# foundation-model-stack/fms-fsdp

Measured on AMD Instinct MI355X. Metric: tokens/sec (aggregate), higher is better.
Workload: dtype bf16; 1 GPU; model=llama2_7b, global_batch=2, seq_len=4096, parallelism=hsdp1

## Files before the change

fms_fsdp_amd/models/llama.py:

```python

import math
import os
from dataclasses import dataclass


import torch
import torch.nn as nn

from fms_fsdp_amd import ops


@dataclass
class LlamaConfig:
    src_vocab_size: int = 32000
    emb_dim: int = 4096
    nheads: int = 32
    kvheads: int = 0
    nlayers: int = 32
    hidden_grow_factor: float = 8 / 3
    multiple_of: int = 256
    max_expected_seq_len: int = 4096
    rope_theta: float = 10000.0
    norm_eps: float = 1e-6

# ... 101 lines not shown
        v = v.view(b, s, self.kvheads, self.head_dim)
        q, k = ops.rope_apply(q, k, cos, sin)
        if cache is not None:
            import torch.nn.functional as F
            if cache.get("k") is not None:
                k = torch.cat([cache["k"], k], dim=1)
                v = torch.cat([cache["v"], v], dim=1)
            cache["k"], cache["v"] = k, v
            o = F.scaled_dot_product_attention(
                q.transpose(1, 2), k.transpose(1, 2), v.transpose(1, 2),
                is_causal=(s == k.shape[1]),
                enable_gqa=(self.kvheads != self.nheads)).transpose(1, 2)
        else:
            o = ops.attention_causal(q, k, v, doc_mask=doc_mask)
        return self._project_out(o.reshape(b, s, -1), residual, b, s)

    def reset_parameters(self):
        for lin in (self.qkv, self.proj):
            nn.init.trunc_normal_(lin.weight, mean=0.0, std=0.02)


class SwiGLU(nn.Module):
    def __init__(self, cfg: LlamaConfig):
        super().__init__()
        self.hidden_dim = cfg.hidden_dim
        self.wg1 = nn.Linear(cfg.emb_dim, 2 * cfg.hidden_dim, bias=False)
        self.w2 = nn.Linear(cfg.hidden_dim, cfg.emb_dim, bias=False)
        self.wg1.weight._direct_wgrad = True
        self.w2.weight._direct_wgrad = True

    def forward(self, x, residual=None):
        if getattr(self, "_disable_fused_residual", False):
            gu = self.wg1(x)
            h = ops.swiglu(gu)
            out = self.w2(h)
            return out if residual is None else out + residual.view_as(out)
        gu = ops.linear_flat(x, self.wg1.weight)
        h = ops.swiglu(gu)
        return ops.linear_flat(h, self.w2.weight, residual)

    def reset_parameters(self):
        for lin in (self.wg1, self.w2):
            nn.init.trunc_normal_(lin.weight, mean=0.0, std=0.02)


class LlamaBlock(nn.Module):

    def __init__(self, cfg: LlamaConfig):
        super().__init__()
        self.attn_norm = RMSNorm(cfg.emb_dim, cfg.norm_eps)
        self.attn = Attention(cfg)
        self.mlp_norm = RMSNorm(cfg.emb_dim, cfg.norm_eps)
        self.mlp = SwiGLU(cfg)

    def forward(self, x, cos, sin, cache=None, doc_mask=None):
        if cache is None and getattr(self, "_ac_enabled", False) \
                and torch.is_grad_enabled():
            return torch.utils.checkpoint.checkpoint(
                self._forward_impl, x, cos, sin, None, doc_mask,
                use_reentrant=False)
        return self._forward_impl(x, cos, sin, cache, doc_mask)

    def _forward_impl(self, x, cos, sin, cache=None, doc_mask=None):
        h = self.attn(self.attn_norm(x), cos, sin, cache, residual=x,
                      doc_mask=doc_mask)
        return self.mlp(self.mlp_norm(h), residual=h)

    def reset_parameters(self):
        for m in (self.attn_norm, self.attn, self.mlp_norm, self.mlp):
            m.reset_parameters()


class Llama(nn.Module):
    def __init__(self, cfg: LlamaConfig):
        super().__init__()
        self.config = cfg
        self.embedding = nn.Embedding(cfg.src_vocab_size, cfg.emb_dim)
        self.rot_emb = RotaryEmbedding(cfg.head_dim, cfg.max_expected_seq_len, cfg.rope_theta)
        self.layers = nn.ModuleList([LlamaBlock(cfg) for _ in range(cfg.nlayers)])
        self.norm = RMSNorm(cfg.emb_dim, cfg.norm_eps)
        self.lm_head = nn.Linear(cfg.emb_dim, cfg.src_vocab_size, bias=False)
        self.doc_mask_token = None

    def forward(self, tokens, labels=None, include_embeds=False,
                doc_mask=None):
        b, s = tokens.shape
        if doc_mask is None and self.doc_mask_token is not None:
            doc_mask = ops.doc_mask_from_tokens(tokens, self.doc_mask_token)
        x = self.embedding(tokens)
        cos, sin = self.rot_emb.get(s, x.device)
        for layer in self.layers:
            x = layer(x, cos, sin, doc_mask=doc_mask)
        x = self.norm(x)
        if labels is not None:
            loss = ops.linear_cross_entropy(x, self.lm_head.weight, labels)
            return (loss, x) if include_embeds else loss
        logits = self.lm_head(x)
        return (logits, x) if include_embeds else logits

    @torch.no_grad()
    def generate(self, input_ids, max_new_tokens, temperature=1.0,
                 do_sample=True, include_embeds=False):
        b, s0 = input_ids.shape
        caches = [{} for _ in self.layers]
        tokens = input_ids
        embeds = []
        cur = input_ids
        pos = 0
        for step in range(max_new_tokens):
            x = self.embedding(cur)
            total = pos + cur.shape[1]
            cos, sin = self.rot_emb.get(total, x.device)
            cos_c, sin_c = cos[pos:total], sin[pos:total]
            for layer, cache in zip(self.layers, caches):
                x = layer(x, cos_c, sin_c, cache)
            x = self.norm(x)
            h_last = x[:, -1:]
            logits = self.lm_head(h_last)[:, -1]
            if do_sample:
                probs = torch.softmax(logits.float() / temperature, dim=-1)
                nxt = torch.multinomial(probs, 1)
            else:
                nxt = logits.argmax(-1, keepdim=True)
            embeds.append(h_last)
            tokens = torch.cat([tokens, nxt], dim=1)
            pos = total
            cur = nxt
        if include_embeds:
            return tokens, torch.cat(embeds, dim=1)
        return tokens

    def reset_root_parameters(self):
        nn.init.trunc_normal_(self.embedding.weight, mean=0.0, std=0.02)
# ... 11 lines not shown
```

fms_fsdp_amd/ops/__init__.py:

```python

import os
from typing import NamedTuple

import torch

from . import reference


_C = None
_C_err = None
try:
    from fms_fsdp_amd import _C
except ImportError as e:
    _C_err = e


def _require_ext(op):
    if _C is None:
        raise RuntimeError(
            f"fms_fsdp_amd._C HIP extension is required for {op} on GPU but "
            f"could not be imported ({_C_err}). Build it with "
            f"`python setup.py build_ext --inplace` (PYTORCH_ROCM_ARCH=gfx950)."
        )
    return _C


class _RMSNormFn(torch.autograd.Function):
    @staticmethod
    def forward(ctx, x, weight, eps):
        ext = _require_ext("rmsnorm")
        x2d = x.contiguous().view(-1, x.shape[-1])
        y, rinv = ext.rmsnorm_fwd(x2d, weight, eps)
        ctx.save_for_backward(x2d, weight, rinv)
        ctx.shape = x.shape
        return y.view(x.shape)

    @staticmethod
    def backward(ctx, dy):
        x2d, weight, rinv = ctx.saved_tensors
        dx, dw = _C.rmsnorm_bwd(dy.contiguous().view_as(x2d), x2d, weight,
                                rinv, None)
        return dx.view(ctx.shape), dw.to(weight.dtype), None


def rmsnorm(x, weight, eps=1e-6):
    if x.is_cuda and x.dtype != torch.float32:
        if x.dtype == torch.float16:
            return _RMSNormFn.apply(x.bfloat16(), weight.bfloat16(),
                                    eps).half()
        return _RMSNormFn.apply(x, weight, eps)
    return reference.rmsnorm(x, weight, eps)


class _AddRMSNormFn(torch.autograd.Function):

    @staticmethod
    def forward(ctx, x, res, weight, eps):
        ext = _require_ext("add_rmsnorm")
        x2d = x.contiguous().view(-1, x.shape[-1])
        r2d = res.contiguous().view_as(x2d)
        y, s, rinv = ext.add_rmsnorm_fwd(x2d, r2d, weight, eps)
        ctx.save_for_backward(s, weight, rinv)
        ctx.shape = x.shape
        return y.view(x.shape), s.view(x.shape)

    @staticmethod
    def backward(ctx, dy, ds):
        s, weight, rinv = ctx.saved_tensors
        dx, dw = _C.rmsnorm_bwd(dy.contiguous().view_as(s), s, weight, rinv,
                                ds.contiguous().view_as(s))
        dx = dx.view(ctx.shape)
        return dx, dx, dw.to(weight.dtype), None


def add_rmsnorm(x, res, weight, eps=1e-6):
    if x.is_cuda and x.dtype != torch.float32:
        if x.dtype == torch.float16:
            y, s = _AddRMSNormFn.apply(x.bfloat16(), res.bfloat16(),
                                       weight.bfloat16(), eps)
            return y.half(), s.half()
        return _AddRMSNormFn.apply(x, res, weight, eps)
    s = (x.float() + res.float()).to(x.dtype)
    return reference.rmsnorm(s, weight, eps), s


def _row_view_ok(t):
    return (t.dim() == 4 and t.stride(3) == 1 and t.stride(2) == t.shape[3]
            and t.stride(1) >= t.shape[2] * t.shape[3]
            and t.stride(0) == t.shape[1] * t.stride(1))


def _as_row_view(t):
    return t if _row_view_ok(t) else t.contiguous()


class _RoPEFn(torch.autograd.Function):
    @staticmethod
    def forward(ctx, q, k, cos, sin):
        ext = _require_ext("rope")
        cos = cos.float().contiguous()
        sin = sin.float().contiguous()
        qo, ko = ext.rope_fwd(_as_row_view(q), _as_row_view(k), cos, sin,
                              False)
        ctx.save_for_backward(cos, sin)
# ... 477 lines not shown
```

fms_fsdp_amd/ops/hip/attention.hip:

```cpp
#include <cstdlib>
#include <cstring>

#include "common.h"
#include "attn_sched.h"
#include "attn_ws.h"

typedef __attribute__((ext_vector_type(8))) __bf16 bf16x8v;
typedef __attribute__((ext_vector_type(16))) float f32x16;
typedef __attribute__((ext_vector_type(4))) float f32x4v;

union U8 {
  bf16x8v v;
  unsigned u[4];
  bf16x8 s;
};

__device__ __forceinline__ unsigned pack2(float lo, float hi) {
  return ((unsigned)(unsigned short)f2bf(hi) << 16) |
         (unsigned short)f2bf(lo);
}

__device__ __forceinline__ bf16x8v pack_pT_chunk(const float* p) {
  unsigned w01 = pack2(p[0], p[1]);
  unsigned w23 = pack2(p[2], p[3]);
// ... 288 lines not shown
    if (act1) {
      const unsigned pvbase = pvb[cur] + 1024;
      U2x64 fr[2][2];
      tr_issue4<0, 128, 512, 640>(pvbase, fr[0][0], fr[0][1]);
#pragma unroll
      for (int t = 0; t < NT; ++t) {
        const int pp = t & 1;
        if (t + 1 < NT) {
          if (t + 1 == 1)
            tr_issue4<4096, 4096 + 128, 4096 + 512, 4096 + 640>(
                pvbase, fr[1][0], fr[1][1]);
          else if (t + 1 == 2)
            tr_issue4<8192, 8192 + 128, 8192 + 512, 8192 + 640>(
                pvbase, fr[0][0], fr[0][1]);
          else
            tr_issue4<12288, 12288 + 128, 12288 + 512, 12288 + 640>(
                pvbase, fr[1][0], fr[1][1]);
          tr_wait<4>(fr[pp][0], fr[pp][1]);
        } else {
          tr_wait<0>(fr[pp][0], fr[pp][1]);
        }
        accO[t] = __builtin_amdgcn_mfma_f32_32x32x16_bf16(fr[pp][0].v, pb1_0,
                                                          accO[t], 0, 0, 0);
        accO[t] = __builtin_amdgcn_mfma_f32_32x32x16_bf16(fr[pp][1].v, pb1_1,
                                                          accO[t], 0, 0, 0);
      }
    }
    __syncthreads();
    cur ^= 1;
  }

  const float inv_l = 1.f / l_run;
  short* op = og + ((long long)b * S * H + (long long)h) * D +
              (long long)my_q * qrow_stride;
#pragma unroll
  for (int t = 0; t < NT; ++t) {
#pragma unroll
    for (int g = 0; g < 4; ++g) {
      const int dv0 = t * 32 + 8 * g + 4 * hb;
      bf16x4 w;
#pragma unroll
      for (int j = 0; j < 4; ++j)
        w.v[j] = f2bf(accO[t][g * 4 + j] * inv_l);
      *(bf16x4*)(op + dv0) = w;
    }
  }
  if (hb == 0)
    lseg[((long long)bh) * S + my_q] =
        (m_run + __log2f(l_run)) * 0.6931471805599453f;
}
#undef KLDS
#undef VLDS

__global__ void attn_bwd_delta_kernel(const short* __restrict__ dog,
                                      const short* __restrict__ og,
                                      float* __restrict__ delta,
                                      int D, int S, int H, long long rows) {
  const long long row = ((long long)blockIdx.x * blockDim.x + threadIdx.x) / 64;
  if (row >= rows) return;
  const int lane = threadIdx.x & 63;
  const short* dop = dog + row * D;
  const short* op = og + row * D;
  float acc = 0.f;
  for (int i = lane * 2; i < D; i += 128) {
    acc += bf2f(dop[i]) * bf2f(op[i]) + bf2f(dop[i + 1]) * bf2f(op[i + 1]);
  }
  acc = wave_reduce_sum(acc);
  if (lane == 0) {
    const long long b = row / ((long long)S * H);
    const int si = (int)((row / H) % S);
    const int hi = (int)(row % H);
    delta[(b * H + hi) * (long long)S + si] = acc;
  }
}

template <int D>
__global__ __launch_bounds__(256, 2) void attn_bwd_dq_kernel(
    const short* __restrict__ kg, const short* __restrict__ dsw,
    short* __restrict__ dqg, int B, int S, int H, int KVH, int sched,
    int ws_tiled) {
  constexpr int KVB = 32;
  constexpr int NT = D / 32;
  extern __shared__ __attribute__((aligned(16))) char smem[];
  constexpr int KIMGB = KVB * D * 2;
  constexpr int SIMGB = KVB * 128 * 2;
#define KIMG(buf) (smem + ((buf) ? KIMGB + SIMGB : 0))
#define SIMG(buf) (smem + KIMGB + ((buf) ? KIMGB + SIMGB : 0))

  const int lane = threadIdx.x & 63;
  const int wid = threadIdx.x >> 6;
  const int col = lane & 31;
  const int hb = lane >> 5;

  const AttnWork wk = attn_sched_map(blockIdx.x, S / 128, B * H, sched, false);
  const int bh = __builtin_amdgcn_readfirstlane(wk.bh);
  const int b = bh / H;
  const int h = bh % H;
  const int kvh = h / (H / KVH);
  const int q0 = __builtin_amdgcn_readfirstlane(wk.tile) * 128;
  const int qw = q0 + wid * 32;
  const int my_q = qw + col;

  const long long qrow_stride = (long long)H * D;
  const long long krow_stride = (long long)KVH * D;
  const short* kbase = kg + ((long long)b * S * KVH + (long long)kvh) * D;
  const short* dsbase = dsw + (long long)bh * S * S + q0;

  f32x16 accDQ[NT];
#pragma unroll
  for (int t = 0; t < NT; ++t) accDQ[t] = (f32x16)(0.f);

  const int ntiles = (q0 + 128 + KVB - 1) / KVB;
  const int t256 = threadIdx.x;
  const int skey = t256 & 31;
  const int sgrp = t256 >> 5;
  const int skd0 = sgrp * (D / 8);
  const short* kp_s = kbase + (long long)skey * krow_stride + skd0;
  const long long kstep = (long long)KVB * krow_stride;
  const short* sp_s =
      ws_tiled ? dsw + (long long)bh * S * S +
                     (long long)(q0 / 32 + (sgrp >> 1)) * 1024 +
// ... 855 lines not shown
  attn_bwd_dkv_keylane_kernel<D, OUT, false, true>                            \
      <<<grid, 256, lds_dkv, stream>>>(                                       \
          (const short*)do_, (const short*)q, (const short*)k,                \
          (const short*)v, lse, delta_ws, dk, dv, (short*)nullptr, B, S, H,   \
          KVH, scale, vstride, dvstride, sched, 0, doc_end)
  if (out_bf16)
    DKV_DOC_LAUNCH(true);
  else
    DKV_DOC_LAUNCH(false);
#undef DKV_DOC_LAUNCH
  const int lds_dq = 2 * (32 * D * 2 + 32 * D * 2);
  attn_bwd_dq_recompute_kernel<D, true><<<grid, 256, lds_dq, stream>>>(
      (const short*)do_, (const short*)q, (const short*)k, (const short*)v,
      lse, delta_ws, (short*)dq, B, S, H, KVH, scale, vstride, sched,
      doc_start);
}

extern "C" {

long long attn_bwd_ws_limit(long long bytes) {
  const long long prev = attn_ws_limit_get();
  if (bytes >= 0) g_attn_ws_limit = bytes;
  return prev;
}

int attn_sched_mode(int mode) {
  const int prev = attn_sched_get();
  if (mode >= 0) g_attn_sched = mode;
  return prev;
}

int attn_dkv_mode(int mode) {
  const int prev = attn_dkv_get();
  if (mode >= 0) g_attn_dkv = mode;
  return prev;
}

void launch_attn_fwd(const void* q, const void* k, const void* v, void* o,
                     float* lse, int B, int S, int H, int KVH, int D,
                     float scale, long long vstride, hipStream_t stream) {
  const unsigned grid = (unsigned)(S / 128) * (unsigned)(B * H);
  const int sched = attn_sched_get();
  const int lds = 3 * 64 * D * 2;
  if (D == 128)
    attn_fwd_kernel<128><<<grid, 256, lds, stream>>>(
        (const short*)q, (const short*)k, (const short*)v, (short*)o, lse, B,
        S, H, KVH, scale, vstride, sched);
  else
    attn_fwd_kernel<64><<<grid, 256, lds, stream>>>(
        (const short*)q, (const short*)k, (const short*)v, (short*)o, lse, B,
        S, H, KVH, scale, vstride, sched);
}

void launch_attn_bwd(const void* do_, const void* q, const void* k,
                     const void* v, const void* o, const float* lse, void* dq,
                     void* dk, void* dv, float* delta_ws, void* ds_ws,
                     int B, int S, int H,
                     int KVH, int D, float scale, int out_bf16,
                     long long vstride, long long dvstride,
                     hipStream_t stream) {
  const long long rows = (long long)B * S * H;
  attn_bwd_delta_kernel<<<(int)((rows * 64 + 255) / 256), 256, 0, stream>>>(
      (const short*)do_, (const short*)o, delta_ws, D, S, H, rows);
  if (D == 128)
    attn_bwd_launch<128>(do_, q, k, v, lse, dq, dk, dv, delta_ws, ds_ws, B, S,
                         H, KVH, scale, out_bf16, vstride, dvstride, stream);
  else
    attn_bwd_launch<64>(do_, q, k, v, lse, dq, dk, dv, delta_ws, ds_ws, B, S,
                        H, KVH, scale, out_bf16, vstride, dvstride, stream);
}

void launch_attn_fwd_doc(const void* q, const void* k, const void* v, void* o,
                         float* lse, const int* doc_start, int B, int S,
                         int H, int KVH, int D, float scale,
                         long long vstride, hipStream_t stream) {
  const unsigned grid = (unsigned)(S / 128) * (unsigned)(B * H);
  const int sched = attn_sched_get();
  const int lds = 3 * 64 * D * 2;
  if (D == 128)
    attn_fwd_kernel<128, true><<<grid, 256, lds, stream>>>(
        (const short*)q, (const short*)k, (const short*)v, (short*)o, lse, B,
        S, H, KVH, scale, vstride, sched, doc_start);
  else
    attn_fwd_kernel<64, true><<<grid, 256, lds, stream>>>(
        (const short*)q, (const short*)k, (const short*)v, (short*)o, lse, B,
        S, H, KVH, scale, vstride, sched, doc_start);
}

void launch_attn_bwd_doc(const void* do_, const void* q, const void* k,
                         const void* v, const void* o, const float* lse,
                         void* dq, void* dk, void* dv, float* delta_ws,
                         const int* doc_start, const int* doc_end, int B,
                         int S, int H, int KVH, int D, float scale,
                         int out_bf16, long long vstride, long long dvstride,
                         hipStream_t stream) {
  const long long rows = (long long)B * S * H;
  attn_bwd_delta_kernel<<<(int)((rows * 64 + 255) / 256), 256, 0, stream>>>(
      (const short*)do_, (const short*)o, delta_ws, D, S, H, rows);
  if (D == 128)
    attn_bwd_doc_launch<128>(do_, q, k, v, lse, dq, dk, dv, delta_ws,
                             doc_start, doc_end, B, S, H, KVH, scale,
                             out_bf16, vstride, dvstride, stream);
  else
    attn_bwd_doc_launch<64>(do_, q, k, v, lse, dq, dk, dv, delta_ws,
                            doc_start, doc_end, B, S, H, KVH, scale,
                            out_bf16, vstride, dvstride, stream);
}

}
```

fms_fsdp_amd/ops/hip/bindings.cpp:

```cpp
#include <torch/extension.h>
#include <c10/hip/HIPStream.h>
#include <hip/hip_runtime_api.h>

#include <string>
#include <tuple>
#include <vector>

#include "attn_ws.h"

using torch::Tensor;

extern "C" {
void launch_rmsnorm_fwd(const void*, const void*, void*, float*, int, int,
                        float, hipStream_t);
void launch_rmsnorm_bwd(const void*, const void*, const void*, const float*,
                        const void*, void*, float*, int, int, hipStream_t);
void launch_add_rmsnorm_fwd(const void*, const void*, const void*, void*,
                            void*, float*, int, int, float, hipStream_t);
void launch_rope(const void*, void*, const float*, const float*, int, int,
                 int, int, int, long long, long long, hipStream_t);
void launch_swiglu_fwd(const void*, void*, long long, int, hipStream_t);
void launch_swiglu_bwd(const void*, const void*, void*, long long, int,
                       hipStream_t);
void launch_ce_fwd_bwd(void*, const long long*, float*, const float*,
                       long long, int, int, hipStream_t);
void launch_adamw(float*, const void*, int, float*, float*, void*, int,
                  long long, float, float, float, float, float, float, float,
                  const float*, hipStream_t);
void launch_sqnorm(const void*, int, float*, long long, hipStream_t);
void launch_attn_fwd(const void*, const void*, const void*, void*, float*,
                     int, int, int, int, int, float, long long, hipStream_t);
void launch_attn_bwd(const void*, const void*, const void*, const void*,
                     const void*, const float*, void*, void*, void*, float*,
                     void*, int, int, int, int, int, float, int,
                     long long, long long, hipStream_t);
void launch_attn_fwd_doc(const void*, const void*, const void*, void*, float*,
                         const int*, int, int, int, int, int, float,
                         long long, hipStream_t);
void launch_attn_bwd_doc(const void*, const void*, const void*, const void*,
                         const void*, const float*, void*, void*, void*,
                         float*, const int*, const int*, int, int, int, int,
                         int, float, int, long long, long long, hipStream_t);
int attn_sched_mode(int);
int attn_dkv_mode(int);
long long attn_bwd_ws_limit(long long);
void launch_cconv_fwd(const void*, const void*, const float*, void*, int,
                      int, int, int, hipStream_t);
void launch_cconv_bwd(const void*, const void*, const void*, const float*,
                      void*, void*, float*, float*, int, int, int, int,
                      hipStream_t);
int launch_gemm_nt(const void*, const void*, void*, int, int, int,
                   hipStream_t);
void launch_segsum_exp_fwd(const float*, void*, long long, int, hipStream_t);
void launch_segsum_exp_bwd(const void*, const float*, float*, long long, int,
                           hipStream_t);
void launch_ssd_prep_fwd(const void*, const float*, const float*, float*,
                         float*, long long, int, int, long long, hipStream_t);
void launch_ssd_prep_bwd(const float*, const float*, const void*,
                         const float*, const float*, void*, float*, float*,
                         long long, int, int, long long, long long,
                         hipStream_t);
void launch_ssd_xdt_fwd(const void*, const float*, const float*, void*, void*,
                        long long, int, int, int, long long, hipStream_t);
void launch_ssd_xdt_bwd(const void*, const void*, const void*, const float*,
                        const float*, void*, float*, float*, long long, int,
                        int, int, long long, long long, hipStream_t);
void launch_ssd_sl_fwd(const float*, const void*, void*, long long, int, int,
                       int, hipStream_t);
void launch_ssd_sl_bwd(const void*, const void*, const float*, void*, float*,
                       long long, int, int, int, hipStream_t);
void launch_ssd_ygate_fwd(const void*, const void*, const float*, const void*,
                          const float*, const void*, void*, long long, int,
                          int, int, int, long long, long long, hipStream_t);
void launch_ssd_ygate_bwd(const void*, const void*, const void*, const float*,
                          const void*, const float*, const void*, void*,
                          void*, float*, void*, float*, void*, long long, int,
                          int, int, int, long long, long long, long long,
                          long long, hipStream_t);
}

static hipStream_t cur_stream() {
  return c10::hip::getCurrentHIPStream().stream();
}

#define CHECK_BF16_CONTIG(t)                                        \
  TORCH_CHECK(t.scalar_type() == torch::kBFloat16, #t " must be bf16"); \
  TORCH_CHECK(t.is_contiguous(), #t " must be contiguous");

std::tuple<Tensor, Tensor> rmsnorm_fwd(Tensor x, Tensor w, double eps) {
  CHECK_BF16_CONTIG(x);
  CHECK_BF16_CONTIG(w);
  const int rows = x.size(0), H = x.size(1);
  TORCH_CHECK(H % 8 == 0, "H must be divisible by 8");
  auto y = torch::empty_like(x);
  auto rinv = torch::empty({rows}, x.options().dtype(torch::kFloat32));
  launch_rmsnorm_fwd(x.data_ptr(), w.data_ptr(), y.data_ptr(),
                     rinv.data_ptr<float>(), rows, H, (float)eps,
                     cur_stream());
  return {y, rinv};
}

std::tuple<Tensor, Tensor> rmsnorm_bwd(Tensor dy, Tensor x, Tensor w,
                                       Tensor rinv,
                                       c10::optional<Tensor> dextra) {
  CHECK_BF16_CONTIG(dy);
  CHECK_BF16_CONTIG(x);
  CHECK_BF16_CONTIG(w);
  TORCH_CHECK(x.dim() == 2 && dy.sizes() == x.sizes(),
              "dy and x must be (rows, H)");
  const int rows = x.size(0), H = x.size(1);
  TORCH_CHECK(H % 8 == 0, "H must be divisible by 8");
  TORCH_CHECK(w.numel() == H, "w must have H elements");
  TORCH_CHECK(rinv.scalar_type() == torch::kFloat32 && rinv.is_contiguous() &&
                  rinv.numel() == rows,
              "rinv must be fp32 with one element per row");
  if (dextra.has_value()) {
    TORCH_CHECK(dextra->scalar_type() == torch::kBFloat16 &&
                    dextra->is_contiguous() && dextra->sizes() == x.sizes(),
                "dextra must have x's shape and dtype");
  }
  auto dx = torch::empty_like(x);
  auto dw = torch::zeros({H}, x.options().dtype(torch::kFloat32));
  launch_rmsnorm_bwd(dy.data_ptr(), x.data_ptr(), w.data_ptr(),
                     rinv.data_ptr<float>(),
                     dextra.has_value() ? dextra->data_ptr() : nullptr,
                     dx.data_ptr(), dw.data_ptr<float>(), rows, H,
                     cur_stream());
  return {dx, dw};
}

std::tuple<Tensor, Tensor, Tensor> add_rmsnorm_fwd(Tensor x, Tensor res,
                                                   Tensor w, double eps) {
  CHECK_BF16_CONTIG(x);
  CHECK_BF16_CONTIG(res);
  const int rows = x.size(0), H = x.size(1);
  auto y = torch::empty_like(x);
  auto s_out = torch::empty_like(x);
  auto rinv = torch::empty({rows}, x.options().dtype(torch::kFloat32));
  launch_add_rmsnorm_fwd(x.data_ptr(), res.data_ptr(), w.data_ptr(),
                         y.data_ptr(), s_out.data_ptr(),
                         rinv.data_ptr<float>(), rows, H, (float)eps,
                         cur_stream());
  return {y, s_out, rinv};
}

static long long row_stride4(const Tensor& t) {
  TORCH_CHECK(t.scalar_type() == torch::kBFloat16, "expected bf16");
  TORCH_CHECK(t.dim() == 4 && t.stride(3) == 1 &&
                  t.stride(2) == t.size(3) &&
                  t.stride(1) >= t.size(2) * t.size(3) &&
                  t.stride(0) == t.size(1) * t.stride(1),
              "expected row-contiguous (b,s,h,d) view");
  return (long long)t.stride(1);
}

std::tuple<Tensor, Tensor> rope_fwd(Tensor q, Tensor k, Tensor cos,
                                    Tensor sin, bool conj) {
  TORCH_CHECK(cos.scalar_type() == torch::kFloat32 && cos.is_contiguous());
  const int b = q.size(0), s = q.size(1), h = q.size(2), d = q.size(3);
  const int kvh = k.size(2);
  const long long qs = row_stride4(q), ks = row_stride4(k);
  TORCH_CHECK((d / 2) % 4 == 0, "head_dim/2 must be divisible by 4");
  auto qo = torch::empty({b, s, h, d}, q.options());
  auto ko = torch::empty({b, s, kvh, d}, k.options());
  launch_rope(q.data_ptr(), qo.data_ptr(), cos.data_ptr<float>(),
              sin.data_ptr<float>(), b, s, h, d, conj, qs,
              (long long)h * d, cur_stream());
  launch_rope(k.data_ptr(), ko.data_ptr(), cos.data_ptr<float>(),
              sin.data_ptr<float>(), b, s, kvh, d, conj, ks,
              (long long)kvh * d, cur_stream());
  return {qo, ko};
}

void rope_into(Tensor src, Tensor dst, Tensor cos, Tensor sin, bool conj) {
  const int b = src.size(0), s = src.size(1), h = src.size(2),
            d = src.size(3);
  const long long is = row_stride4(src), os = row_stride4(dst);
  TORCH_CHECK(dst.size(2) == h && dst.size(3) == d);
  launch_rope(src.data_ptr(), dst.data_ptr(), cos.data_ptr<float>(),
              sin.data_ptr<float>(), b, s, h, d, conj, is, os,
              cur_stream());
// ... 126 lines not shown
std::tuple<Tensor, Tensor> attn_fwd(Tensor q, Tensor k, Tensor v) {
  CHECK_BF16_CONTIG(q);
  CHECK_BF16_CONTIG(k);
  const long long vs = row_stride4(v);
  const int b = q.size(0), s = q.size(1), h = q.size(2), d = q.size(3);
  const int kvh = k.size(2);
  TORCH_CHECK(d == 64 || d == 128, "head_dim must be 64 or 128");
  TORCH_CHECK(s % 128 == 0, "seq len must be a multiple of 128");
  auto o = torch::empty_like(q);
  auto lse = torch::empty({b, h, s}, q.options().dtype(torch::kFloat32));
  const float scale = 1.f / sqrtf((float)d);
  launch_attn_fwd(q.data_ptr(), k.data_ptr(), v.data_ptr(), o.data_ptr(),
                  lse.data_ptr<float>(), b, s, h, kvh, d, scale, vs,
                  cur_stream());
  return {o, lse};
}

std::tuple<Tensor, Tensor, Tensor> attn_bwd(Tensor do_, Tensor q, Tensor k,
                                            Tensor v, Tensor o, Tensor lse,
                                            c10::optional<Tensor> dv_out) {
  CHECK_BF16_CONTIG(do_);
  const long long vs = row_stride4(v);
  const int b = q.size(0), s = q.size(1), h = q.size(2), d = q.size(3);
  const int kvh = k.size(2);
  auto dq = torch::empty_like(q);
  const bool out_bf16 = (kvh == h);
  auto opts = q.options().dtype(out_bf16 ? torch::kBFloat16 : torch::kFloat32);
  auto dk = out_bf16 ? torch::empty({b, s, kvh, d}, opts)
                     : torch::zeros({b, s, kvh, d}, opts);
  Tensor dv;
  long long dvs = (long long)kvh * d;
  if (dv_out.has_value() && out_bf16) {
    dv = *dv_out;
    dvs = row_stride4(dv);
  } else {
    dv = out_bf16 ? torch::empty({b, s, kvh, d}, opts)
                  : torch::zeros({b, s, kvh, d}, opts);
  }
  auto delta = torch::empty({b, h, s}, q.options().dtype(torch::kFloat32));
  Tensor ds_ws;
  if (attn_bwd_use_workspace(b, h, s, attn_bwd_ws_limit(-1)))
    ds_ws = torch::empty({(long long)b * h, (long long)s, (long long)s},
                         q.options());
  const float scale = 1.f / sqrtf((float)d);
  launch_attn_bwd(do_.data_ptr(), q.data_ptr(), k.data_ptr(), v.data_ptr(),
                  o.data_ptr(), lse.data_ptr<float>(), dq.data_ptr(),
                  dk.data_ptr(), dv.data_ptr(), delta.data_ptr<float>(),
                  ds_ws.defined() ? ds_ws.data_ptr() : nullptr, b, s,
                  h, kvh, d, scale, out_bf16 ? 1 : 0, vs, dvs, cur_stream());
  if (out_bf16) return {dq, dk, dv};
  return {dq, dk.to(torch::kBFloat16), dv.to(torch::kBFloat16)};
}

static void check_doc_array(const Tensor& t, const Tensor& q,
                            const char* name) {
  TORCH_CHECK(t.scalar_type() == torch::kInt32, name, " must be int32");
  TORCH_CHECK(t.is_contiguous(), name, " must be contiguous");
  TORCH_CHECK(t.dim() == 2 && t.size(0) == q.size(0) && t.size(1) == q.size(1),
              name, " must have shape (b, s)");
  TORCH_CHECK(t.device() == q.device(), name, " must be on q's device");
}

std::tuple<Tensor, Tensor> attn_fwd_doc(Tensor q, Tensor k, Tensor v,
                                        Tensor doc_start) {
  CHECK_BF16_CONTIG(q);
  CHECK_BF16_CONTIG(k);
  const long long vs = row_stride4(v);
  const int b = q.size(0), s = q.size(1), h = q.size(2), d = q.size(3);
  const int kvh = k.size(2);
  TORCH_CHECK(d == 64 || d == 128, "head_dim must be 64 or 128");
  TORCH_CHECK(s % 128 == 0, "seq len must be a multiple of 128");
  check_doc_array(doc_start, q, "doc_start");
  auto o = torch::empty_like(q);
  auto lse = torch::empty({b, h, s}, q.options().dtype(torch::kFloat32));
  const float scale = 1.f / sqrtf((float)d);
  launch_attn_fwd_doc(q.data_ptr(), k.data_ptr(), v.data_ptr(), o.data_ptr(),
                      lse.data_ptr<float>(), doc_start.data_ptr<int>(), b, s,
                      h, kvh, d, scale, vs, cur_stream());
  return {o, lse};
}

std::tuple<Tensor, Tensor, Tensor> attn_bwd_doc(
    Tensor do_, Tensor q, Tensor k, Tensor v, Tensor o, Tensor lse,
    c10::optional<Tensor> dv_out, Tensor doc_start, Tensor doc_end) {
  CHECK_BF16_CONTIG(do_);
  const long long vs = row_stride4(v);
  const int b = q.size(0), s = q.size(1), h = q.size(2), d = q.size(3);
  const int kvh = k.size(2);
  check_doc_array(doc_start, q, "doc_start");
  check_doc_array(doc_end, q, "doc_end");
  auto dq = torch::empty_like(q);
  const bool out_bf16 = (kvh == h);
  auto opts = q.options().dtype(out_bf16 ? torch::kBFloat16 : torch::kFloat32);
  auto dk = out_bf16 ? torch::empty({b, s, kvh, d}, opts)
                     : torch::zeros({b, s, kvh, d}, opts);
  Tensor dv;
  long long dvs = (long long)kvh * d;
  if (dv_out.has_value() && out_bf16) {
    dv = *dv_out;
    dvs = row_stride4(dv);
  } else {
    dv = out_bf16 ? torch::empty({b, s, kvh, d}, opts)
                  : torch::zeros({b, s, kvh, d}, opts);
  }
  auto delta = torch::empty({b, h, s}, q.options().dtype(torch::kFloat32));
  const float scale = 1.f / sqrtf((float)d);
// ... 247 lines not shown
  check_nq(dacs, x.size(0) / Q * H, Q, "dacs");
  check_head_vec(Dp, H, "D");
}

Tensor ssd_ygate_fwd(Tensor ydiag, Tensor yoff, Tensor dacs, Tensor x,
                     Tensor Dp, Tensor z, int64_t H, int64_t G, int64_t P,
                     int64_t Q) {
  const long long sx = check_xslice(x, H, P, Q, "x");
  const long long sz = check_xslice(z, H, P, Q, "z");
  const long long rows = x.size(0);
  check_ygate(ydiag, yoff, dacs, x, Dp, z, H, G, Q);
  auto out = torch::empty({rows, H * P}, x.options().dtype(torch::kBFloat16));
  launch_ssd_ygate_fwd(ydiag.data_ptr(), yoff.data_ptr(),
                       dacs.data_ptr<float>(), x.data_ptr(),
                       Dp.data_ptr<float>(), z.data_ptr(), out.data_ptr(),
                       rows * H * P / 8, (int)H, (int)G, (int)Q, (int)P, sx,
                       sz, cur_stream());
  return out;
}

std::vector<Tensor> ssd_ygate_bwd(Tensor dout, Tensor ydiag, Tensor yoff,
                                  Tensor dacs, Tensor x, Tensor Dp, Tensor z,
                                  int64_t H, int64_t G, int64_t P,
                                  int64_t Q) {
  const long long sx = check_xslice(x, H, P, Q, "x");
  const long long sz = check_xslice(z, H, P, Q, "z");
  const long long rows = x.size(0);
  check_ygate(ydiag, yoff, dacs, x, Dp, z, H, G, Q);
  check_bf16_numel(dout, rows * H * P, "dout");
  auto o = x.options().dtype(torch::kBFloat16);
  auto dydiag = torch::empty({rows, H * P}, o);
  auto dyoff = torch::empty({rows, H * P}, o);
  auto ddacs = torch::empty_like(dacs);
  auto dx = torch::empty({rows, H * P}, o);
  auto dD_rows = torch::empty({rows, H}, x.options().dtype(torch::kFloat32));
  auto dz = torch::empty({rows, H * P}, o);
  launch_ssd_ygate_bwd(dout.data_ptr(), ydiag.data_ptr(), yoff.data_ptr(),
                       dacs.data_ptr<float>(), x.data_ptr(),
                       Dp.data_ptr<float>(), z.data_ptr(), dydiag.data_ptr(),
                       dyoff.data_ptr(), ddacs.data_ptr<float>(),
                       dx.data_ptr(), dD_rows.data_ptr<float>(),
                       dz.data_ptr(), rows * H, (int)H, (int)G, (int)Q,
                       (int)P, sx, sz, H * P, H * P, cur_stream());
  return {dydiag, dyoff, ddacs, dx, dD_rows, dz};
}

PYBIND11_MODULE(TORCH_EXTENSION_NAME, mod) {
  mod.def("segsum_exp_fwd", &segsum_exp_fwd);
  mod.def("segsum_exp_bwd", &segsum_exp_bwd);
  mod.def("cconv_fwd", &cconv_fwd);
  mod.def("cconv_bwd", &cconv_bwd);
  mod.def("rmsnorm_fwd", &rmsnorm_fwd);
  mod.def("rmsnorm_bwd", &rmsnorm_bwd);
  mod.def("add_rmsnorm_fwd", &add_rmsnorm_fwd);
  mod.def("rope_fwd", &rope_fwd);
  mod.def("rope_into", &rope_into);
  mod.def("swiglu_fwd", &swiglu_fwd);
  mod.def("swiglu_bwd", &swiglu_bwd);
  mod.def("ce_fwd_bwd", &ce_fwd_bwd);
  mod.def("adamw", &adamw);
  mod.def("sq_norm_accum", &sq_norm_accum);
  mod.def("gemm_nt", &gemm_nt);
  mod.def("ssd_prep_fwd", &ssd_prep_fwd);
  mod.def("ssd_prep_bwd", &ssd_prep_bwd);
  mod.def("ssd_xdt_fwd", &ssd_xdt_fwd);
  mod.def("ssd_xdt_bwd", &ssd_xdt_bwd);
  mod.def("ssd_sl_fwd", &ssd_sl_fwd);
  mod.def("ssd_sl_bwd", &ssd_sl_bwd);
  mod.def("ssd_ygate_fwd", &ssd_ygate_fwd);
  mod.def("ssd_ygate_bwd", &ssd_ygate_bwd);
  mod.def("attn_fwd", &attn_fwd);
  mod.def("attn_bwd", &attn_bwd);
  mod.def("attn_fwd_doc", &attn_fwd_doc);
  mod.def("attn_bwd_doc", &attn_bwd_doc);
  mod.def("attn_sched_mode", &attn_sched_mode_py,
          pybind11::arg("mode") = pybind11::none());
  mod.def("attn_dkv_mode", &attn_dkv_mode_py,
          pybind11::arg("mode") = pybind11::none());
  mod.def("attn_bwd_ws_limit", &attn_bwd_ws_limit_py,
          pybind11::arg("bytes") = pybind11::none());
}
```

fms_fsdp_amd/ops/hip/rmsnorm.hip:

```cpp
#include "common.h"

__global__ void rmsnorm_fwd_kernel(const bf16x8* __restrict__ x,
                                   const bf16x8* __restrict__ w,
                                   bf16x8* __restrict__ y,
                                   float* __restrict__ rinv,
                                   int H8, float eps, int rows) {
  __shared__ float scratch[16];
  for (int row = blockIdx.x; row < rows; row += gridDim.x) {
    const bf16x8* xr = x + (size_t)row * H8;
    bf16x8* yr = y + (size_t)row * H8;
    float ss = 0.f;
    for (int i = threadIdx.x; i < H8; i += blockDim.x) {
      bf16x8 v = xr[i];
#pragma unroll
      for (int j = 0; j < 8; ++j) {
        float f = bf2f(v.v[j]);
        ss += f * f;
      }
    }
    ss = block_reduce_sum(ss, scratch);
    float r = rsqrtf(ss / (H8 * 8) + eps);
    if (threadIdx.x == 0) rinv[row] = r;
    for (int i = threadIdx.x; i < H8; i += blockDim.x) {
      bf16x8 v = xr[i];
// ... 61 lines not shown
  __shared__ float scratch[16];
  const int H = H8 * 8;
  for (int row = blockIdx.x; row < rows; row += gridDim.x) {
    const bf16x8* dyr = dy + (size_t)row * H8;
    const bf16x8* xr = x + (size_t)row * H8;
    bf16x8* dxr = dx + (size_t)row * H8;
    const float r = rinv[row];
    float s = 0.f;
    for (int i = threadIdx.x; i < H8; i += blockDim.x) {
      bf16x8 d = dyr[i], xv = xr[i], wv = w[i];
#pragma unroll
      for (int j = 0; j < 8; ++j)
        s += bf2f(d.v[j]) * bf2f(wv.v[j]) * bf2f(xv.v[j]);
    }
    s = block_reduce_sum(s, scratch);
    const float c = r * r * r * s / H;
    for (int i = threadIdx.x; i < H8; i += blockDim.x) {
      bf16x8 d = dyr[i], xv = xr[i], wv = w[i];
      bf16x8 o;
      if (dextra != nullptr) {
        const bf16x8 de = dextra[(size_t)row * H8 + i];
#pragma unroll
        for (int j = 0; j < 8; ++j)
          o.v[j] = f2bf(r * bf2f(wv.v[j]) * bf2f(d.v[j]) - c * bf2f(xv.v[j])
                        + bf2f(de.v[j]));
      } else {
#pragma unroll
        for (int j = 0; j < 8; ++j)
          o.v[j] = f2bf(r * bf2f(wv.v[j]) * bf2f(d.v[j]) - c * bf2f(xv.v[j]));
      }
      dxr[i] = o;
    }
    __syncthreads();
  }
}

__global__ void rmsnorm_bwd_dw_kernel(const short* __restrict__ dy,
                                      const short* __restrict__ x,
                                      const float* __restrict__ rinv,
                                      float* __restrict__ dw,
                                      int H, int rows, int rows_per_chunk) {
  const int col = blockIdx.x * blockDim.x + threadIdx.x;
  if (col >= H) return;
  const int r0 = blockIdx.y * rows_per_chunk;
  const int r1 = min(r0 + rows_per_chunk, rows);
  float acc = 0.f;
  for (int i = r0; i < r1; ++i) {
    size_t off = (size_t)i * H + col;
    acc += bf2f(dy[off]) * bf2f(x[off]) * rinv[i];
  }
  atomicAdd(&dw[col], acc);
}

extern "C" {

void launch_rmsnorm_fwd(const void* x, const void* w, void* y, float* rinv,
                        int rows, int H, float eps, hipStream_t stream) {
  int grid = min(rows, 2048);
  rmsnorm_fwd_kernel<<<grid, 256, 0, stream>>>(
      (const bf16x8*)x, (const bf16x8*)w, (bf16x8*)y, rinv, H / 8, eps, rows);
}

void launch_add_rmsnorm_fwd(const void* x, const void* res, const void* w,
                            void* y, void* s_out, float* rinv, int rows,
                            int H, float eps, hipStream_t stream) {
  int grid = min(rows, 2048);
  add_rmsnorm_fwd_kernel<<<grid, 256, 0, stream>>>(
      (const bf16x8*)x, (const bf16x8*)res, (const bf16x8*)w, (bf16x8*)y,
      (bf16x8*)s_out, rinv, H / 8, eps, rows);
}

void launch_rmsnorm_bwd(const void* dy, const void* x, const void* w,
                        const float* rinv, const void* dextra, void* dx,
                        float* dw, int rows, int H, hipStream_t stream) {
  int grid = min(rows, 2048);
  rmsnorm_bwd_dx_kernel<<<grid, 256, 0, stream>>>(
      (const bf16x8*)dy, (const bf16x8*)x, (const bf16x8*)w, rinv,
      (const bf16x8*)dextra, (bf16x8*)dx, H / 8, rows);
  int rows_per_chunk = max(1, (rows + 63) / 64);
  dim3 g2((H + 255) / 256, (rows + rows_per_chunk - 1) / rows_per_chunk);
  rmsnorm_bwd_dw_kernel<<<g2, 256, 0, stream>>>(
      (const short*)dy, (const short*)x, rinv, dw, H, rows, rows_per_chunk);
}

}
```

Measured before the change: 22490 tokens/s.

## Fuse RMSNorm backward dx/dw, write wgrad directly, vectorize attention delta

Replaces the two-kernel RMSNorm backward (dx pass plus atomic column dw pass) with a single fused kernel that keeps weights and per-block dw partials in registers, followed by a small finalize reduction. When a parameter exposes a flat grad view, it writes bf16 dw straight into it to skip a separate grad copy. The norm residual output is routed back through the norm's own backward so dres is folded in via dextra. The attention backward delta kernel is also vectorized to use 16 or 8 lanes per row with bf16x8 loads instead of a full wave per row. The direct-wgrad path depends on _flat_grad_view being set externally, and the extra partial buffers add memory traffic.

```diff
diff --git a/fms_fsdp_amd/models/llama.py b/fms_fsdp_amd/models/llama.py
--- a/fms_fsdp_amd/models/llama.py
+++ b/fms_fsdp_amd/models/llama.py
@@ -177,6 +177,8 @@
         self.attn = Attention(cfg)
         self.mlp_norm = RMSNorm(cfg.emb_dim, cfg.norm_eps)
         self.mlp = SwiGLU(cfg)
+        self.attn_norm.weight._direct_wgrad = True
+        self.mlp_norm.weight._direct_wgrad = True
 
     def forward(self, x, cos, sin, cache=None, doc_mask=None):
         if cache is None and getattr(self, "_ac_enabled", False) \
@@ -187,9 +189,12 @@
         return self._forward_impl(x, cos, sin, cache, doc_mask)
 
     def _forward_impl(self, x, cos, sin, cache=None, doc_mask=None):
-        h = self.attn(self.attn_norm(x), cos, sin, cache, residual=x,
-                      doc_mask=doc_mask)
-        return self.mlp(self.mlp_norm(h), residual=h)
+        n, x_res = ops.rmsnorm_residual(x, self.attn_norm.weight,
+                                        self.attn_norm.eps)
+        h = self.attn(n, cos, sin, cache, residual=x_res, doc_mask=doc_mask)
+        n, h_res = ops.rmsnorm_residual(h, self.mlp_norm.weight,
+                                        self.mlp_norm.eps)
+        return self.mlp(n, residual=h_res)
 
     def reset_parameters(self):
         for m in (self.attn_norm, self.attn, self.mlp_norm, self.mlp):
@@ -204,6 +209,7 @@
         self.rot_emb = RotaryEmbedding(cfg.head_dim, cfg.max_expected_seq_len, cfg.rope_theta)
         self.layers = nn.ModuleList([LlamaBlock(cfg) for _ in range(cfg.nlayers)])
         self.norm = RMSNorm(cfg.emb_dim, cfg.norm_eps)
+        self.norm.weight._direct_wgrad = True
         self.lm_head = nn.Linear(cfg.emb_dim, cfg.src_vocab_size, bias=False)
         self.doc_mask_token = None
 
diff --git a/fms_fsdp_amd/ops/__init__.py b/fms_fsdp_amd/ops/__init__.py
--- a/fms_fsdp_amd/ops/__init__.py
+++ b/fms_fsdp_amd/ops/__init__.py
@@ -25,31 +25,129 @@
     return _C
 
 
+def _direct_wgrad_on(weight):
+    return (getattr(weight, "_flat_grad_view", None) is not None
+            and weight.requires_grad and torch.is_grad_enabled())
+
+
+def _stash_wgrad_target(ctx, weight):
+    ctx.gview = weight._flat_grad_view
+    ctx.wobj = weight
+    ctx.cb = getattr(weight, "_wgrad_done", None)
+
+
+def _take_wgrad_fresh(ctx):
+    fresh = getattr(ctx.wobj, "_wgrad_fresh", False)
+    ctx.wobj._wgrad_fresh = False
+    return fresh
+
+
+class _WgradSinkFn(torch.autograd.Function):
+
+    @staticmethod
+    def forward(ctx, weight):
+        _stash_wgrad_target(ctx, weight)
+        return weight.view_as(weight)
+
+    @staticmethod
+    def backward(ctx, dw):
+        if _take_wgrad_fresh(ctx):
+            ctx.gview.copy_(dw)
+        else:
+            ctx.gview.add_(dw)
+        if ctx.cb is not None:
+            ctx.cb()
+        return None
+
+
+def _rmsnorm_backward(ctx, dy, dextra):
+    x2d, weight, rinv = ctx.saved_tensors
+    if dy is None:
+        dy = torch.zeros_like(x2d)
+    dy = dy.contiguous().view_as(x2d)
+    if dextra is not None:
+        dextra = dextra.contiguous().view_as(x2d)
+    if ctx.direct:
+        dx = _C.rmsnorm_bwd_into(dy, x2d, weight, rinv, dextra,
+                                 ctx.gview.view(-1),
+                                 not _take_wgrad_fresh(ctx))
+        if ctx.cb is not None:
+            ctx.cb()
+        return dx.view(ctx.shape), None
+    dx, dw = _C.rmsnorm_bwd(dy, x2d, weight, rinv, dextra)
+    return dx.view(ctx.shape), dw.to(weight.dtype)
+
+
 class _RMSNormFn(torch.autograd.Function):
     @staticmethod
-    def forward(ctx, x, weight, eps):
+    def forward(ctx, x, weight, eps, direct=False):
         ext = _require_ext("rmsnorm")
         x2d = x.contiguous().view(-1, x.shape[-1])
         y, rinv = ext.rmsnorm_fwd(x2d, weight, eps)
         ctx.save_for_backward(x2d, weight, rinv)
         ctx.shape = x.shape
+        ctx.direct = direct
+        if direct:
+            _stash_wgrad_target(ctx, weight)
         return y.view(x.shape)
 
     @staticmethod
     def backward(ctx, dy):
-        x2d, weight, rinv = ctx.saved_tensors
-        dx, dw = _C.rmsnorm_bwd(dy.contiguous().view_as(x2d), x2d, weight,
-                                rinv, None)
-        return dx.view(ctx.shape), dw.to(weight.dtype), None
+        dx, dw = _rmsnorm_backward(ctx, dy, None)
+        return dx, dw, None, None
+
+
+class _RMSNormResidualFn(torch.autograd.Function):
+
+    @staticmethod
+    def forward(ctx, x, weight, eps, direct=False):
+        ext = _require_ext("rmsnorm")
+        x2d = x.contiguous().view(-1, x.shape[-1])
+        y, rinv = ext.rmsnorm_fwd(x2d, weight, eps)
+        ctx.save_for_backward(x2d, weight, rinv)
+        ctx.shape = x.shape
+        ctx.direct = direct
+        if direct:
+            _stash_wgrad_target(ctx, weight)
+        ctx.set_materialize_grads(False)
+        return y.view(x.shape), x2d.view(x.shape)
+
+    @staticmethod
+    def backward(ctx, dy, dres):
+        dx, dw = _rmsnorm_backward(ctx, dy, dres)
+        return dx, dw, None, None
+
+
+def _rmsnorm_dispatch(fn, x, weight, eps):
+    if not (x.is_cuda and x.dtype != torch.float32):
+        return None
+    if x.dtype == torch.float16:
+        if _direct_wgrad_on(weight):
+            weight = _WgradSinkFn.apply(weight)
+        y = _RMSNormFn.apply(x.bfloat16(), weight.bfloat16(), eps).half()
+        return y if fn is _RMSNormFn else (y, x)
+    direct = _direct_wgrad_on(weight) and weight.dtype == torch.bfloat16
+    if not direct and _direct_wgrad_on(weight):
+        weight = _WgradSinkFn.apply(weight)
+    return fn.apply(x, weight, eps, direct)
 
 
 def rmsnorm(x, weight, eps=1e-6):
-    if x.is_cuda and x.dtype != torch.float32:
-        if x.dtype == torch.float16:
-            return _RMSNormFn.apply(x.bfloat16(), weight.bfloat16(),
-                                    eps).half()
-        return _RMSNormFn.apply(x, weight, eps)
+    y = _rmsnorm_dispatch(_RMSNormFn, x, weight, eps)
+    if y is not None:
+        return y
+    if _direct_wgrad_on(weight):
+        weight = _WgradSinkFn.apply(weight)
     return reference.rmsnorm(x, weight, eps)
+
+
+def rmsnorm_residual(x, weight, eps=1e-6):
+    out = _rmsnorm_dispatch(_RMSNormResidualFn, x, weight, eps)
+    if out is not None:
+        return out
+    if _direct_wgrad_on(weight):
+        weight = _WgradSinkFn.apply(weight)
+    return reference.rmsnorm(x, weight, eps), x
 
 
 class _AddRMSNormFn(torch.autograd.Function):
diff --git a/fms_fsdp_amd/ops/hip/attention.hip b/fms_fsdp_amd/ops/hip/attention.hip
--- a/fms_fsdp_amd/ops/hip/attention.hip
+++ b/fms_fsdp_amd/ops/hip/attention.hip
@@ -364,21 +364,22 @@
 #undef KLDS
 #undef VLDS
 
-__global__ void attn_bwd_delta_kernel(const short* __restrict__ dog,
-                                      const short* __restrict__ og,
-                                      float* __restrict__ delta,
-                                      int D, int S, int H, long long rows) {
-  const long long row = ((long long)blockIdx.x * blockDim.x + threadIdx.x) / 64;
-  if (row >= rows) return;
-  const int lane = threadIdx.x & 63;
-  const short* dop = dog + row * D;
-  const short* op = og + row * D;
+template <int LPR>
+__global__ __launch_bounds__(256) void attn_bwd_delta_kernel(
+    const bf16x8* __restrict__ dog, const bf16x8* __restrict__ og,
+    float* __restrict__ delta, int S, int H, long long rows) {
+  const long long gid = (long long)blockIdx.x * blockDim.x + threadIdx.x;
+  const long long row = gid / LPR;
   float acc = 0.f;
-  for (int i = lane * 2; i < D; i += 128) {
-    acc += bf2f(dop[i]) * bf2f(op[i]) + bf2f(dop[i + 1]) * bf2f(op[i + 1]);
-  }
-  acc = wave_reduce_sum(acc);
-  if (lane == 0) {
+  if (row < rows) {
+    const bf16x8 a = dog[gid], c = og[gid];
+#pragma unroll
+    for (int j = 0; j < 8; ++j) acc += bf2f(a.v[j]) * bf2f(c.v[j]);
+  }
+#pragma unroll
+  for (int off = LPR / 2; off > 0; off >>= 1)
+    acc += __shfl_xor(acc, off, LPR);
+  if (row < rows && (threadIdx.x & (LPR - 1)) == 0) {
     const long long b = row / ((long long)S * H);
     const int si = (int)((row / H) % S);
     const int hi = (int)(row % H);
@@ -1340,6 +1341,18 @@
         S, H, KVH, scale, vstride, sched);
 }
 
+void launch_attn_bwd_delta(const void* do_, const void* o, float* delta,
+                           int B, int S, int H, int D, hipStream_t stream) {
+  const long long rows = (long long)B * S * H;
+  const unsigned grid = (unsigned)((rows * (D / 8) + 255) / 256);
+  if (D == 128)
+    attn_bwd_delta_kernel<16><<<grid, 256, 0, stream>>>(
+        (const bf16x8*)do_, (const bf16x8*)o, delta, S, H, rows);
+  else
+    attn_bwd_delta_kernel<8><<<grid, 256, 0, stream>>>(
+        (const bf16x8*)do_, (const bf16x8*)o, delta, S, H, rows);
+}
+
 void launch_attn_bwd(const void* do_, const void* q, const void* k,
                      const void* v, const void* o, const float* lse, void* dq,
                      void* dk, void* dv, float* delta_ws, void* ds_ws,
@@ -1347,9 +1360,7 @@
                      int KVH, int D, float scale, int out_bf16,
                      long long vstride, long long dvstride,
                      hipStream_t stream) {
-  const long long rows = (long long)B * S * H;
-  attn_bwd_delta_kernel<<<(int)((rows * 64 + 255) / 256), 256, 0, stream>>>(
-      (const short*)do_, (const short*)o, delta_ws, D, S, H, rows);
+  launch_attn_bwd_delta(do_, o, delta_ws, B, S, H, D, stream);
   if (D == 128)
     attn_bwd_launch<128>(do_, q, k, v, lse, dq, dk, dv, delta_ws, ds_ws, B, S,
                          H, KVH, scale, out_bf16, vstride, dvstride, stream);
@@ -1382,9 +1393,7 @@
                          int S, int H, int KVH, int D, float scale,
                          int out_bf16, long long vstride, long long dvstride,
                          hipStream_t stream) {
-  const long long rows = (long long)B * S * H;
-  attn_bwd_delta_kernel<<<(int)((rows * 64 + 255) / 256), 256, 0, stream>>>(
-      (const short*)do_, (const short*)o, delta_ws, D, S, H, rows);
+  launch_attn_bwd_delta(do_, o, delta_ws, B, S, H, D, stream);
   if (D == 128)
     attn_bwd_doc_launch<128>(do_, q, k, v, lse, dq, dk, dv, delta_ws,
                              doc_start, doc_end, B, S, H, KVH, scale,
diff --git a/fms_fsdp_amd/ops/hip/bindings.cpp b/fms_fsdp_amd/ops/hip/bindings.cpp
--- a/fms_fsdp_amd/ops/hip/bindings.cpp
+++ b/fms_fsdp_amd/ops/hip/bindings.cpp
@@ -17,6 +17,12 @@
                         const void*, void*, float*, int, int, hipStream_t);
 void launch_add_rmsnorm_fwd(const void*, const void*, const void*, void*,
                             void*, float*, int, int, float, hipStream_t);
+int rmsnorm_bwd_grid(int);
+int rmsnorm_bwd_nparts(int, int);
+void launch_rmsnorm_bwd_fused(const void*, const void*, const void*,
+                              const float*, const void*, void*, float*, int,
+                              float*, void*, int, int, int, hipStream_t);
+void launch_rmsnorm_dw_store(const float*, void*, int, int, hipStream_t);
 void launch_rope(const void*, void*, const float*, const float*, int, int,
                  int, int, int, long long, long long, hipStream_t);
 void launch_swiglu_fwd(const void*, void*, long long, int, hipStream_t);
@@ -41,6 +47,8 @@
                          const void*, const float*, void*, void*, void*,
                          float*, const int*, const int*, int, int, int, int,
                          int, float, int, long long, long long, hipStream_t);
+void launch_attn_bwd_delta(const void*, const void*, float*, int, int, int,
+                           int, hipStream_t);
 int attn_sched_mode(int);
 int attn_dkv_mode(int);
 long long attn_bwd_ws_limit(long long);
@@ -100,9 +108,9 @@
   return {y, rinv};
 }
 
-std::tuple<Tensor, Tensor> rmsnorm_bwd(Tensor dy, Tensor x, Tensor w,
-                                       Tensor rinv,
-                                       c10::optional<Tensor> dextra) {
+static void check_rmsnorm_bwd_args(const Tensor& dy, const Tensor& x,
+                                   const Tensor& w, const Tensor& rinv,
+                                   const c10::optional<Tensor>& dextra) {
   CHECK_BF16_CONTIG(dy);
   CHECK_BF16_CONTIG(x);
   CHECK_BF16_CONTIG(w);
@@ -119,14 +127,70 @@
                     dextra->is_contiguous() && dextra->sizes() == x.sizes(),
                 "dextra must have x's shape and dtype");
   }
+}
+
+std::tuple<Tensor, Tensor> rmsnorm_bwd(Tensor dy, Tensor x, Tensor w,
+                                       Tensor rinv,
+                                       c10::optional<Tensor> dextra) {
+  check_rmsnorm_bwd_args(dy, x, w, rinv, dextra);
+  const int rows = x.size(0), H = x.size(1);
+  const void* de = dextra.has_value() ? dextra->data_ptr() : nullptr;
+  auto f32 = x.options().dtype(torch::kFloat32);
   auto dx = torch::empty_like(x);
-  auto dw = torch::zeros({H}, x.options().dtype(torch::kFloat32));
-  launch_rmsnorm_bwd(dy.data_ptr(), x.data_ptr(), w.data_ptr(),
-                     rinv.data_ptr<float>(),
-                     dextra.has_value() ? dextra->data_ptr() : nullptr,
-                     dx.data_ptr(), dw.data_ptr<float>(), rows, H,
-                     cur_stream());
+  const int nparts = rmsnorm_bwd_nparts(rows, H);
+  if (nparts == 0) {
+    auto dw = torch::zeros({H}, f32);
+    launch_rmsnorm_bwd(dy.data_ptr(), x.data_ptr(), w.data_ptr(),
+                       rinv.data_ptr<float>(), de, dx.data_ptr(),
+                       dw.data_ptr<float>(), rows, H, cur_stream());
+    return {dx, dw};
+  }
+  auto dw = torch::empty({H}, f32);
+  auto part = torch::empty({nparts, H}, f32);
+  launch_rmsnorm_bwd_fused(dy.data_ptr(), x.data_ptr(), w.data_ptr(),
+                           rinv.data_ptr<float>(), de, dx.data_ptr(),
+                           part.data_ptr<float>(), nparts,
+                           dw.data_ptr<float>(), nullptr, 0, rows, H,
+                           cur_stream());
   return {dx, dw};
+}
+
+Tensor rmsnorm_bwd_into(Tensor dy, Tensor x, Tensor w, Tensor rinv,
+                        c10::optional<Tensor> dextra, Tensor dw_dst,
+                        bool accumulate) {
+  check_rmsnorm_bwd_args(dy, x, w, rinv, dextra);
+  const int rows = x.size(0), H = x.size(1);
+  TORCH_CHECK(dw_dst.scalar_type() == torch::kBFloat16 &&
+                  dw_dst.is_contiguous() && dw_dst.numel() == H &&
+                  dw_dst.device() == x.device(),
+              "dw_dst must be contiguous bf16 with H elements on x's device");
+  const void* de = dextra.has_value() ? dextra->data_ptr() : nullptr;
+  auto f32 = x.options().dtype(torch::kFloat32);
+  auto dx = torch::empty_like(x);
+  const int mode = accumulate ? 2 : 1;
+  const int nparts = rmsnorm_bwd_nparts(rows, H);
+  if (nparts == 0) {
+    auto dw = torch::zeros({H}, f32);
+    launch_rmsnorm_bwd(dy.data_ptr(), x.data_ptr(), w.data_ptr(),
+                       rinv.data_ptr<float>(), de, dx.data_ptr(),
+                       dw.data_ptr<float>(), rows, H, cur_stream());
+    launch_rmsnorm_dw_store(dw.data_ptr<float>(), dw_dst.data_ptr(), mode, H,
+                            cur_stream());
+    return dx;
+  }
+  auto part = torch::empty({nparts, H}, f32);
+  launch_rmsnorm_bwd_fused(dy.data_ptr(), x.data_ptr(), w.data_ptr(),
+                           rinv.data_ptr<float>(), de, dx.data_ptr(),
+                           part.data_ptr<float>(), nparts, nullptr,
+                           dw_dst.data_ptr(), mode, rows, H, cur_stream());
+  return dx;
+}
+
+int64_t rmsnorm_bwd_grid_py(c10::optional<int64_t> grid) {
+  if (grid.has_value())
+    TORCH_CHECK(*grid >= 1 && *grid <= 65536,
+                "rmsnorm_bwd_grid: expected 1..65536, got ", *grid);
+  return rmsnorm_bwd_grid(grid.has_value() ? (int)*grid : -1);
 }
 
 std::tuple<Tensor, Tensor, Tensor> add_rmsnorm_fwd(Tensor x, Tensor res,
@@ -359,6 +423,19 @@
   return {dq, dk.to(torch::kBFloat16), dv.to(torch::kBFloat16)};
 }
 
+Tensor attn_bwd_delta(Tensor do_, Tensor o) {
+  CHECK_BF16_CONTIG(do_);
+  CHECK_BF16_CONTIG(o);
+  TORCH_CHECK(do_.dim() == 4 && do_.sizes() == o.sizes(),
+              "do and o must be (b, s, h, d) of one shape");
+  const int b = o.size(0), s = o.size(1), h = o.size(2), d = o.size(3);
+  TORCH_CHECK(d == 64 || d == 128, "head_dim must be 64 or 128");
+  auto delta = torch::empty({b, h, s}, o.options().dtype(torch::kFloat32));
+  launch_attn_bwd_delta(do_.data_ptr(), o.data_ptr(), delta.data_ptr<float>(),
+                        b, s, h, d, cur_stream());
+  return delta;
+}
+
 static void check_doc_array(const Tensor& t, const Tensor& q,
                             const char* name) {
   TORCH_CHECK(t.scalar_type() == torch::kInt32, name, " must be int32");
@@ -712,6 +789,9 @@
   mod.def("cconv_bwd", &cconv_bwd);
   mod.def("rmsnorm_fwd", &rmsnorm_fwd);
   mod.def("rmsnorm_bwd", &rmsnorm_bwd);
+  mod.def("rmsnorm_bwd_into", &rmsnorm_bwd_into);
+  mod.def("rmsnorm_bwd_grid", &rmsnorm_bwd_grid_py,
+          pybind11::arg("grid") = pybind11::none());
   mod.def("add_rmsnorm_fwd", &add_rmsnorm_fwd);
   mod.def("rope_fwd", &rope_fwd);
   mod.def("rope_into", &rope_into);
@@ -731,6 +811,7 @@
   mod.def("ssd_ygate_bwd", &ssd_ygate_bwd);
   mod.def("attn_fwd", &attn_fwd);
   mod.def("attn_bwd", &attn_bwd);
+  mod.def("attn_bwd_delta", &attn_bwd_delta);
   mod.def("attn_fwd_doc", &attn_fwd_doc);
   mod.def("attn_bwd_doc", &attn_bwd_doc);
   mod.def("attn_sched_mode", &attn_sched_mode_py,
diff --git a/fms_fsdp_amd/ops/hip/rmsnorm.hip b/fms_fsdp_amd/ops/hip/rmsnorm.hip
--- a/fms_fsdp_amd/ops/hip/rmsnorm.hip
+++ b/fms_fsdp_amd/ops/hip/rmsnorm.hip
@@ -137,7 +137,158 @@
   atomicAdd(&dw[col], acc);
 }
 
+template <int NC>
+__global__ __launch_bounds__(256) void rmsnorm_bwd_fused_kernel(
+    const bf16x8* __restrict__ dy, const bf16x8* __restrict__ x,
+    const bf16x8* __restrict__ w, const float* __restrict__ rinv,
+    const bf16x8* __restrict__ dextra, bf16x8* __restrict__ dx,
+    float* __restrict__ part, int H8, int rows) {
+  __shared__ float scratch[16];
+  const int H = H8 * 8;
+  bf16x8 wv[NC];
+  float pw[NC][8];
+#pragma unroll
+  for (int k = 0; k < NC; ++k) {
+    const int i = threadIdx.x + k * 256;
+    if (i < H8) wv[k] = w[i];
+#pragma unroll
+    for (int j = 0; j < 8; ++j) pw[k][j] = 0.f;
+  }
+  for (int row = blockIdx.x; row < rows; row += gridDim.x) {
+    const bf16x8* dyr = dy + (size_t)row * H8;
+    const bf16x8* xr = x + (size_t)row * H8;
+    bf16x8* dxr = dx + (size_t)row * H8;
+    const float r = rinv[row];
+    bf16x8 d[NC], xv[NC];
+    float s = 0.f;
+#pragma unroll
+    for (int k = 0; k < NC; ++k) {
+      const int i = threadIdx.x + k * 256;
+      if (i < H8) {
+        d[k] = dyr[i];
+        xv[k] = xr[i];
+#pragma unroll
+        for (int j = 0; j < 8; ++j)
+          s += bf2f(d[k].v[j]) * bf2f(wv[k].v[j]) * bf2f(xv[k].v[j]);
+      }
+    }
+    s = block_reduce_sum(s, scratch);
+    const float c = r * r * r * s / H;
+#pragma unroll
+    for (int k = 0; k < NC; ++k) {
+      const int i = threadIdx.x + k * 256;
+      if (i < H8) {
+        bf16x8 o;
+        if (dextra != nullptr) {
+          const bf16x8 de = dextra[(size_t)row * H8 + i];
+#pragma unroll
+          for (int j = 0; j < 8; ++j)
+            o.v[j] = f2bf(r * bf2f(wv[k].v[j]) * bf2f(d[k].v[j]) -
+                          c * bf2f(xv[k].v[j]) + bf2f(de.v[j]));
+        } else {
+#pragma unroll
+          for (int j = 0; j < 8; ++j)
+            o.v[j] = f2bf(r * bf2f(wv[k].v[j]) * bf2f(d[k].v[j]) -
+                          c * bf2f(xv[k].v[j]));
+        }
+        dxr[i] = o;
+#pragma unroll
+        for (int j = 0; j < 8; ++j)
+          pw[k][j] += bf2f(d[k].v[j]) * bf2f(xv[k].v[j]) * r;
+      }
+    }
+    __syncthreads();
+  }
+  f32x4* prow = (f32x4*)(part + (size_t)blockIdx.x * H);
+#pragma unroll
+  for (int k = 0; k < NC; ++k) {
+    const int i = threadIdx.x + k * 256;
+    if (i < H8) {
+      f32x4 lo, hi;
+#pragma unroll
+      for (int j = 0; j < 4; ++j) {
+        lo.v[j] = pw[k][j];
+        hi.v[j] = pw[k][4 + j];
+      }
+      prow[2 * i] = lo;
+      prow[2 * i + 1] = hi;
+    }
+  }
+}
+
+#define RMS_FIN_COLS 16
+#define RMS_FIN_SLICES 16
+__global__ __launch_bounds__(256) void rmsnorm_bwd_dw_finalize_kernel(
+    const float* __restrict__ part, float* __restrict__ dw_f32,
+    short* __restrict__ dw_bf, int H, int nparts, int mode) {
+  __shared__ float red[RMS_FIN_SLICES][RMS_FIN_COLS];
+  const int cl = threadIdx.x % RMS_FIN_COLS;
+  const int sl = threadIdx.x / RMS_FIN_COLS;
+  const int col = blockIdx.x * RMS_FIN_COLS + cl;
+  float acc = 0.f;
+  if (col < H) {
+#pragma unroll 8
+    for (int g = sl; g < nparts; g += RMS_FIN_SLICES)
+      acc += part[(size_t)g * H + col];
+  }
+  red[sl][cl] = acc;
+  __syncthreads();
+  if (sl == 0 && col < H) {
+    float sum = red[0][cl];
+#pragma unroll
+    for (int i = 1; i < RMS_FIN_SLICES; ++i) sum += red[i][cl];
+    if (mode == 0)
+      dw_f32[col] = sum;
+    else if (mode == 1)
+      dw_bf[col] = f2bf(sum);
+    else
+      dw_bf[col] = f2bf(bf2f(dw_bf[col]) + sum);
+  }
+}
+
+static int g_rms_bwd_grid = 1024;
+
 extern "C" {
+
+int rmsnorm_bwd_grid(int grid) {
+  const int prev = g_rms_bwd_grid;
+  if (grid > 0) g_rms_bwd_grid = grid;
+  return prev;
+}
+
+int rmsnorm_bwd_nparts(int rows, int H) {
+  if (H > 8192 || rows <= 0) return 0;
+  return min(rows, g_rms_bwd_grid);
+}
+
+void launch_rmsnorm_bwd_fused(const void* dy, const void* x, const void* w,
+                              const float* rinv, const void* dextra, void* dx,
+                              float* part, int nparts, float* dw_f32,
+                              void* dw_bf, int mode, int rows, int H,
+                              hipStream_t stream) {
+  const int H8 = H / 8;
+#define RMS_FUSED(NC)                                                        \
+  rmsnorm_bwd_fused_kernel<NC><<<nparts, 256, 0, stream>>>(                  \
+      (const bf16x8*)dy, (const bf16x8*)x, (const bf16x8*)w, rinv,           \
+      (const bf16x8*)dextra, (bf16x8*)dx, part, H8, rows)
+  if (H8 <= 256)
+    RMS_FUSED(1);
+  else if (H8 <= 512)
+    RMS_FUSED(2);
+  else
+    RMS_FUSED(4);
+#undef RMS_FUSED
+  rmsnorm_bwd_dw_finalize_kernel<<<(H + RMS_FIN_COLS - 1) / RMS_FIN_COLS, 256,
+                                   0, stream>>>(part, dw_f32, (short*)dw_bf,
+                                                H, nparts, mode);
+}
+
+void launch_rmsnorm_dw_store(const float* dw_f32, void* dw_bf, int mode,
+                             int H, hipStream_t stream) {
+  rmsnorm_bwd_dw_finalize_kernel<<<(H + RMS_FIN_COLS - 1) / RMS_FIN_COLS, 256,
+                                   0, stream>>>(dw_f32, nullptr,
+                                                (short*)dw_bf, H, 1, mode);
+}
 
 void launch_rmsnorm_fwd(const void* x, const void* w, void* y, float* rinv,
                         int rows, int H, float eps, hipStream_t stream) {
```

Result: faster. 22910 tokens/s, median of 6 (+1.9%).
